# x42/meters.lv2

Measured on NVIDIA H100. Metric: audio-samples/sec/GPU (48 kHz stereo, 8192-ch batch) EBU R128 + true-peak, higher is better.
Workload: dtype f32

## Files before the change

### meters.lv2_b200/csrc/tpk.cu

```cuda
#include <math.h>
#include <stdlib.h>
#include <algorithm>
#include "common.cuh"
#include "tpk_internal.cuh"
#include "ebu_kw.cuh"

namespace b200m {

constexpr int TPK_THREADS = 128;

__constant__ float c_tp_tab[120];

struct TpkParams {
    float w1, w2, w3, g;
    float omega, fall; int hold;
    float kq[4], kc4;
};

struct TpkState {
    float *hist;
    float *tp_z1, *tp_z2, *tp_m, *tp_p; int *tp_res;
    float *km_z1, *km_z2, *km_rms, *km_peak, *km_fall; int *km_cnt, *km_fpp, *km_flag;
    unsigned* done_cnt;
    float* hist_alt;
// ... 1159 lines not shown
                    } else fir16<true> (w, xw, o, full0);
                }
                const int nv = min (4, len - 4 * q);
#pragma unroll
                for (int i = 0; i < 4; ++i)
                    if (i < nv) kpv.z = fmax3 (kpv.z, max3_abs (o[4 * i], o[4 * i + 1], o[4 * i + 2]), fabsf (o[4 * i + 3]));
            }
            if (c >= 2) bar_sync_2<BAR_EMPTY, TPK_THREADS> (b);
            if (act) {
                float4* d = reinterpret_cast<float4*> (&ob[b][r][0]);
#pragma unroll
                for (int i = 0; i < 4; ++i)
                    d[i * GPC + q] = make_float4 (fabsf (o[4 * i]), fabsf (o[4 * i + 1]), fabsf (o[4 * i + 2]), fabsf (o[4 * i + 3]));
                kp[b][r][q] = kpv;
            }
            bar_arrive_2<BAR_FULL, TPK_THREADS> (b);
        }
        {
            const int cl = nchunks - 1, base = (cl & (TPD_NSLOT - 1)) * TC + (nfram - cl * TC);
            for (int idx = ftid; idx < CH * 48; idx += TPD_FIR) {
                const int rr = idx / 48, j = idx - 48 * rr;
                if (c0 + rr < n_chan) st.hist[(size_t)(c0 + rr) * 48 + j] = xs[rr][base + j];
            }
        }
    } else {
        const int tch = lane & 15, filt = lane >> 4;
        const int chs = min (c0 + tch, n_chan - 1);
        const bool live = (c0 + tch) < n_chan;
        const int res = st.tp_res[chs];
        float m = res ? 0.0f : st.tp_m[chs];
        float p = res ? 0.0f : st.tp_p[chs];
        float z;
        { const float a = filt ? st.tp_z2[chs] : st.tp_z1[chs]; z = a > 20 ? 20 : (a < 0 ? 0 : a); }
        const float wf = filt ? prm.w2 : prm.w1;
        const float omw = __fsub_rn (1.0f, wf), wq = __fsub_rn (1.0f, omw), omw3 = __fmul_rn (omw, prm.w3);
        float kz1 = 0, kz2 = 0, kt = 0;
        if (KM) {
            const float a = st.km_z1[chs], b = st.km_z2[chs];
            kz1 = a > 50 ? 50 : (a < 0 ? 0 : a);
            kz2 = b > 50 ? 50 : (b < 0 ? 0 : b);
        }
        const float om4 = __fmul_rn (4.0f, prm.omega), nkc4 = -prm.kc4;
        auto step = [&] (const float4 v4) {
            if (FMA) {
                const float zd = __fmul_rn (z, prm.w3);
                z = fmaxf (zd, fmaf (omw3, z, __fmul_rn (wq, v4.x)));
                z = fmaxf (z, fmaf (omw, z, __fmul_rn (wq, v4.y)));
                z = fmaxf (z, fmaf (omw, z, __fmul_rn (wq, v4.z)));
                z = fmaxf (z, fmaf (omw, z, __fmul_rn (wq, v4.w)));
            } else {
                z = __fmul_rn (z, prm.w3);
                if (v4.x > z) z = __fadd_rn (z, __fmul_rn (wf, __fsub_rn (v4.x, z)));
                if (v4.y > z) z = __fadd_rn (z, __fmul_rn (wf, __fsub_rn (v4.y, z)));
                if (v4.z > z) z = __fadd_rn (z, __fmul_rn (wf, __fsub_rn (v4.z, z)));
                if (v4.w > z) z = __fadd_rn (z, __fmul_rn (wf, __fsub_rn (v4.w, z)));
            }
            m = fmaxf (m, __fadd_rn (z, __shfl_xor_sync (0xffffffffu, z, 16)));
        };
        for (int c = 0; c < nchunks; ++c) {
            const int b = c & 1, s0 = c * TC, len = min (TC, nfram - s0);
            bar_sync_2<BAR_FULL, TPK_THREADS> (b);
            const float4* b4 = reinterpret_cast<const float4*> (&ob[b][tch][0]);
            const float4* k4 = &kp[b][tch][0];
            const float4* x4 = reinterpret_cast<const float4*> (&xs[tch][48 + (c & (TPD_NSLOT - 1)) * TC]);
            const int ng = len >> 2;
#pragma unroll 2
            for (int g = 0; g < ng; ++g) {
                const float4 v0 = b4[g], v1 = b4[GPC + g], v2 = b4[2 * GPC + g], v3 = b4[3 * GPC + g];
                const float4 k = k4[g];
                step (v0); step (v1); step (v2); step (v3);
                p = fmaxf (p, k.z);
                if (KM && s0 + 4 * g + 4 <= km_n) {
                    if (FMA) {
                        kz1 = __fadd_rn (kz1, fmaf (nkc4, kz1, k.x));
                        kz2 = fmaf (om4, __fsub_rn (kz1, kz2), kz2);
                        kt = fmaxf (kt, k.y);
                    } else {
                        const float4 xv = x4[g];
                        const float vv[4] = {xv.x, xv.y, xv.z, xv.w};
#pragma unroll
                        for (int i = 0; i < 4; ++i) {
                            const float sq = __fmul_rn (vv[i], vv[i]);
                            if (kt < sq) kt = sq;
                            kz1 = __fadd_rn (kz1, __fmul_rn (prm.omega, __fsub_rn (sq, kz1)));
                        }
                        kz2 = __fadd_rn (kz2, __fmul_rn (om4, __fsub_rn (kz1, kz2)));
                    }
                }
            }
            if (4 * ng < len) {
                for (int j = 4 * ng; j < len; ++j) step (b4[(j & 3) * GPC + (j >> 2)]);
                p = fmaxf (p, k4[ng].z);
            }
            if (c + 2 < nchunks) bar_arrive_2<BAR_EMPTY, TPK_THREADS> (b);
        }
        if (live) {
            if (filt) st.tp_z2[chs] = __fadd_rn (z, 1e-20f);
            else {
                st.tp_z1[chs] = __fadd_rn (z, 1e-20f);
                m = __fmul_rn (m, prm.g);
                if (res) { st.tp_m[chs] = m; st.tp_p[chs] = p; st.tp_res[chs] = 0; }
                else {
                    if (m > st.tp_m[chs]) st.tp_m[chs] = m;
                    if (p > st.tp_p[chs]) st.tp_p[chs] = p;
                }
                if (KM) {
                    if (isnan (kz1)) kz1 = 0;
                    if (isnan (kz2)) kz2 = 0;
                    if (!finitef_ (kt)) kt = 0;
                    st.km_z1[chs] = __fadd_rn (kz1, 1e-20f);
                    st.km_z2[chs] = __fadd_rn (kz2, 1e-20f);
                    const float sr = __fsqrt_rn (__fmul_rn (2.0f, kz2));
                    const float tr = __fsqrt_rn (kt);
                    if (st.km_flag[chs]) { st.km_rms[chs] = sr; st.km_flag[chs] = 0; }
                    else if (sr > st.km_rms[chs]) st.km_rms[chs] = sr;
                    float pk = st.km_peak[chs]; int cnt = st.km_cnt[chs];
                    if (tr >= pk) { pk = tr; cnt = prm.hold; }
                    else if (cnt > 0) cnt -= nfram;
                    else { pk = __fmul_rn (pk, prm.fall); pk = __fadd_rn (pk, 1e-10f); }
                    st.km_peak[chs] = pk; st.km_cnt[chs] = cnt;
                    st.km_fall[chs] = prm.fall; st.km_fpp[chs] = nfram;
                }
            }
        }
    }
}

constexpr int TCF_XPITCH = 308;
constexpr int TCF_XSTAGES = 8;
constexpr int TCF_BLBO = 96 * 16;
constexpr int TCF_BBYTES = 16 * TCF_BLBO;
constexpr int TCF_SMEM = TCF_BBYTES + TCF_XSTAGES * 8 * TCF_XPITCH * 4 + 256;
constexpr int TCF_THREADS = 288;
constexpr int TCF_CONSUMERS = 256;

B200M_DEV uint32_t tcf_smem_u32 (const void* p) { return (uint32_t)__cvta_generic_to_shared (p); }
B200M_DEV uint64_t tcf_desc (uint32_t saddr, uint32_t lbo, uint32_t sbo)
{
    return (uint64_t)((saddr & 0x3FFFFu) >> 4) | ((uint64_t)(lbo >> 4) << 16) | ((uint64_t)(sbo >> 4) << 32);
}
B200M_DEV void tcf_wait (uint32_t bar, uint32_t parity)
{
    uint32_t ok = 0;
    while (!ok) asm volatile ("{ .reg .pred p; mbarrier.try_wait.parity.shared::cta.b64 p, [%1], %2; selp.u32 %0, 1, 0, p; }" : "=r"(ok) : "r"(bar), "r"(parity) : "memory");
}
B200M_DEV void tcf_arrive (uint32_t bar) { asm volatile ("mbarrier.arrive.shared::cta.b64 _, [%0];" :: "r"(bar) : "memory"); }
B200M_DEV void tcf_wgmma_n96 (float (&d)[48], const uint32_t (&a)[4], uint64_t db, uint32_t scale_d)
{
    asm volatile ("{\n\t.reg .pred p;\n\tsetp.ne.b32 p, %53, 0;\n\t"
                  "wgmma.mma_async.sync.aligned.m64n96k8.f32.tf32.tf32 {%0, %1, %2, %3, %4, %5, %6, %7, %8, %9, %10, %11, %12, %13, %14, %15, %16, %17, %18, %19, %20, %21, %22, %23, %24, %25, %26, %27, %28, %29, %30, %31, %32, %33, %34, %35, %36, %37, %38, %39, %40, %41, %42, %43, %44, %45, %46, %47}, {%48, %49, %50, %51}, %52, p, 1, 1;\n\t}\n"
                  : "+f"(d[0]), "+f"(d[1]), "+f"(d[2]), "+f"(d[3]), "+f"(d[4]), "+f"(d[5]), "+f"(d[6]), "+f"(d[7]), "+f"(d[8]), "+f"(d[9]), "+f"(d[10]), "+f"(d[11]), "+f"(d[12]), "+f"(d[13]), "+f"(d[14]), "+f"(d[15]), "+f"(d[16]), "+f"(d[17]), "+f"(d[18]), "+f"(d[19]), "+f"(d[20]), "+f"(d[21]), "+f"(d[22]), "+f"(d[23]), "+f"(d[24]), "+f"(d[25]), "+f"(d[26]), "+f"(d[27]), "+f"(d[28]), "+f"(d[29]), "+f"(d[30]), "+f"(d[31]), "+f"(d[32]), "+f"(d[33]), "+f"(d[34]), "+f"(d[35]), "+f"(d[36]), "+f"(d[37]), "+f"(d[38]), "+f"(d[39]), "+f"(d[40]), "+f"(d[41]), "+f"(d[42]), "+f"(d[43]), "+f"(d[44]), "+f"(d[45]), "+f"(d[46]), "+f"(d[47])
                  : "r"(a[0]), "r"(a[1]), "r"(a[2]), "r"(a[3]), "l"(db), "r"(scale_d) : "memory");
}
B200M_DEV void tcf_wgmma_n48 (float (&d)[48], const uint32_t (&a)[4], uint64_t db, uint32_t scale_d)
{
    asm volatile ("{\n\t.reg .pred p;\n\tsetp.ne.b32 p, %29, 0;\n\t"
                  "wgmma.mma_async.sync.aligned.m64n48k8.f32.tf32.tf32 {%0, %1, %2, %3, %4, %5, %6, %7, %8, %9, %10, %11, %12, %13, %14, %15, %16, %17, %18, %19, %20, %21, %22, %23}, {%24, %25, %26, %27}, %28, p, 1, 1;\n\t}\n"
                  : "+f"(d[0]), "+f"(d[1]), "+f"(d[2]), "+f"(d[3]), "+f"(d[4]), "+f"(d[5]), "+f"(d[6]), "+f"(d[7]), "+f"(d[8]), "+f"(d[9]), "+f"(d[10]), "+f"(d[11]), "+f"(d[12]), "+f"(d[13]), "+f"(d[14]), "+f"(d[15]), "+f"(d[16]), "+f"(d[17]), "+f"(d[18]), "+f"(d[19]), "+f"(d[20]), "+f"(d[21]), "+f"(d[22]), "+f"(d[23])
                  : "r"(a[0]), "r"(a[1]), "r"(a[2]), "r"(a[3]), "l"(db), "r"(scale_d) : "memory");
}

B200M_DEV void tcf_load (const float* xw, float (&v)[8][4])
{
#pragma unroll
    for (int s = 0; s < 8; ++s) { v[s][0] = xw[8 * s]; v[s][1] = xw[16 + 8 * s]; v[s][2] = xw[8 * s + 4]; v[s][3] = xw[16 + 8 * s + 4]; }
}
B200M_DEV float tcf_mask_p0 (float (&v)[8][4], int t, const int (&vj)[2], const int (&nin)[2])
{
    if (nin[1] < 64) {
#pragma unroll
        for (int s = 0; s < 8; ++s)
#pragma unroll
            for (int e = 0; e < 4; ++e)
                if (8 * s + t + 4 * (e >> 1) >= nin[e & 1]) v[s][e] = 0.0f;
    }
    float p0 = 0.0f;
#pragma unroll
    for (int s = 3; s < 5; ++s)
#pragma unroll
        for (int e = 0; e < 4; ++e)
            if (8 * (s - 3) + t + 4 * (e >> 1) < vj[e & 1]) p0 = fmaxf (p0, fabsf (v[s][e]));
    return p0;
}
B200M_DEV void tcf_split (const float (&v)[8][4], uint32_t (&ahi)[8][4], uint32_t (&alo)[8][4])
{
#pragma unroll
    for (int s = 0; s < 8; ++s)
#pragma unroll
        for (int e = 0; e < 4; ++e) {
            const uint32_t hbits = __float_as_uint (v[s][e]) & 0xffffe000u;
            ahi[s][e] = hbits; alo[s][e] = __float_as_uint (__fsub_rn (v[s][e], __uint_as_float (hbits)));
        }
}
B200M_DEV void tcf_mma (float (&d)[48], const uint32_t (&ahi)[8][4], const uint32_t (&alo)[8][4], uint32_t bb)
{
    asm volatile ("wgmma.fence.sync.aligned;" ::: "memory");
#pragma unroll
    for (int s = 0; s < 8; ++s) {
        const uint64_t db = tcf_desc (bb + 2 * s * TCF_BLBO, TCF_BLBO, 128);
        tcf_wgmma_n96 (d, ahi[s], db, s == 0 ? 0u : 1u);
        tcf_wgmma_n48 (d, alo[s], db, 1u);
    }
    asm volatile ("wgmma.commit_group.sync.aligned;" ::: "memory");
}
B200M_DEV void tcf_mma_wait () { asm volatile ("wgmma.wait_group.sync.aligned 0;" ::: "memory"); }
B200M_DEV float tcf_tile_max (const float (&d)[48], int t, const int (&vj)[2], float mx)
{
#pragma unroll
    for (int i = 0; i < 6; ++i)
#pragma unroll
        for (int e = 0; e < 2; ++e) {
            const int j = 8 * (i & 1) + 2 * t + e;
            if (j < vj[0]) mx = fmaxf (mx, fabsf (__fadd_rn (d[4 * i + e], d[4 * (i + 6) + e])));
            if (j < vj[1]) mx = fmaxf (mx, fabsf (__fadd_rn (d[4 * i + 2 + e], d[4 * (i + 6) + 2 + e])));
        }
    return mx;
}

template <int HOLD>
__global__ void __launch_bounds__ (TCF_THREADS, 1)
tpmax_tc_kernel (const float* __restrict__ in, size_t stride, int c_first, int n_chan, int nfram, int nchunks, const float* __restrict__ bcanon,
                 TpkState st, R128Hold r128)
{
    extern __shared__ __align__ (128) uint8_t tcf_smem[];
    uint8_t* sB = tcf_smem;
    float* xbuf = reinterpret_cast<float*> (tcf_smem + TCF_BBYTES);
    uint64_t* bars = reinterpret_cast<uint64_t*> (tcf_smem + TCF_BBYTES + TCF_XSTAGES * 8 * TCF_XPITCH * 4);
    uint64_t* xfull = bars; uint64_t* xempty = bars + TCF_XSTAGES;
    const int tid = threadIdx.x, warp = tid >> 5, lane = tid & 31;
    const int ngroups = (n_chan - c_first + 7) / 8;
    const int n_it = (int)blockIdx.x < ngroups ? ((ngroups - (int)blockIdx.x + (int)gridDim.x - 1) / (int)gridDim.x) * nchunks : 0;
    __shared__ unsigned s_gmax[8];
    if (tid < 8) s_gmax[tid] = 0u;

    for (int i = tid; i < TCF_BBYTES / 16; i += TCF_THREADS) reinterpret_cast<float4*> (sB)[i] = reinterpret_cast<const float4*> (bcanon)[i];
    if (tid == 0) {
        for (int i = 0; i < TCF_XSTAGES; ++i) {
            asm volatile ("mbarrier.init.shared::cta.b64 [%0], 1;" :: "r"(tcf_smem_u32 (&xfull[i])));
            asm volatile ("mbarrier.init.shared::cta.b64 [%0], %1;" :: "r"(tcf_smem_u32 (&xempty[i])), "n"(TCF_CONSUMERS));
        }
        asm volatile ("fence.mbarrier_init.release.cluster;" ::: "memory");
    }
    asm volatile ("fence.proxy.async.shared::cta;" ::: "memory");
    __syncthreads ();

    if (warp == 8) {
        if (lane == 0)
            for (int it = 0; it < n_it; ++it) {
                const int sg = it % TCF_XSTAGES;
                if (it >= TCF_XSTAGES) tcf_wait (tcf_smem_u32 (&xempty[sg]), (uint32_t)((it / TCF_XSTAGES - 1) & 1));
                const int gk = it / nchunks, chunk = it - gk * nchunks;
                const int c0 = c_first + ((int)blockIdx.x + gk * (int)gridDim.x) * 8, s0 = chunk * 256;
                const uint32_t xb = tcf_smem_u32 (xbuf + (size_t)sg * 8 * TCF_XPITCH), bar = tcf_smem_u32 (&xfull[sg]);
                const uint32_t nfl = (uint32_t)min (304, nfram - (s0 - 48));
                asm volatile ("mbarrier.arrive.expect_tx.shared::cta.b64 _, [%0], %1;" :: "r"(bar), "r"(8u * nfl * 4u) : "memory");
                for (int cc = 0; cc < 8; ++cc) {
                    const size_t ch = (size_t)min (c0 + cc, n_chan - 1);
                    const uint32_t dst = xb + (uint32_t)(cc * TCF_XPITCH * 4);
                    if (chunk == 0) {
                        asm volatile ("cp.async.bulk.shared::cluster.global.mbarrier::complete_tx::bytes [%0], [%1], %2, [%3];"
                                      :: "r"(dst), "l"(st.hist + ch * 48), "r"(192u), "r"(bar) : "memory");
                        asm volatile ("cp.async.bulk.shared::cluster.global.mbarrier::complete_tx::bytes [%0], [%1], %2, [%3];"
                                      :: "r"(dst + 192u), "l"(in + ch * stride), "r"((nfl - 48u) * 4u), "r"(bar) : "memory");
                    } else
                        asm volatile ("cp.async.bulk.shared::cluster.global.mbarrier::complete_tx::bytes [%0], [%1], %2, [%3];"
                                      :: "r"(dst), "l"(in + ch * stride + (s0 - 48)), "r"(nfl * 4u), "r"(bar) : "memory");
                }
            }
    } else {
        const int wg = warp >> 2, g = lane >> 2, t = lane & 3;
        const int tb0 = 8 * wg + 2 * (warp & 3);
        const uint32_t bb = tcf_smem_u32 (sB);
        for (int it = 0; it < n_it; ++it) {
            const int gk = it / nchunks, chunk = it - gk * nchunks;
            const int c0 = c_first + ((int)blockIdx.x + gk * (int)gridDim.x) * 8, s0 = chunk * 256;
            const int sg = it % TCF_XSTAGES;
            tcf_wait (tcf_smem_u32 (&xfull[sg]), (uint32_t)((it / TCF_XSTAGES) & 1));
            const float* xt = xbuf + (size_t)sg * 8 * TCF_XPITCH;
            const float* xw = xt + g * TCF_XPITCH + 16 * tb0 + t;
            float v[8][4];
            tcf_load (xw, v);
            if (chunk == nchunks - 1 && tid < 96) {
                const int rr = tid / 12, k4 = (tid - 12 * rr) * 4;
                if (c0 + rr < n_chan)
                    *reinterpret_cast<float4*> (st.hist_alt + (size_t)(c0 + rr) * 48 + k4) = *reinterpret_cast<const float4*> (xt + rr * TCF_XPITCH + (nfram - s0) + k4);
            }
            tcf_arrive (tcf_smem_u32 (&xempty[sg]));
            int vj[2], nin[2];
#pragma unroll
            for (int h = 0; h < 2; ++h) {
                vj[h] = min (16, max (0, nfram - (s0 + 16 * (tb0 + h))));
                nin[h] = nfram - (s0 - 48) - 16 * (tb0 + h);
            }
            const float p0 = tcf_mask_p0 (v, t, vj, nin);
            uint32_t ahi[8][4], alo[8][4];
            tcf_split (v, ahi, alo);
            float d[48];
            tcf_mma (d, ahi, alo, bb);
            tcf_mma_wait ();
            float mx = tcf_tile_max (d, t, vj, p0);
            mx = fmaxf (mx, __shfl_xor_sync (0xffffffffu, mx, 1));
            mx = fmaxf (mx, __shfl_xor_sync (0xffffffffu, mx, 2));
            if (t == 0 && mx > 0.0f) atomicMax (&s_gmax[g], __float_as_uint (mx));
            if (chunk == nchunks - 1) {
                asm volatile ("bar.sync 1, %0;" :: "n"(TCF_CONSUMERS) : "memory");
                if (warp == 0) {
                    const int cc = c0 + lane;
                    const bool own = lane < 8 && cc < n_chan;
                    float mm = 0.0f;
                    if (lane < 8) { const float bm = __uint_as_float (s_gmax[lane]); s_gmax[lane] = 0u; mm = bm; }
                    if (own) {
                        const float m0 = st.tp_res[cc] ? 0.0f : st.tp_m[cc];
                        if (!(mm > m0)) mm = m0;
                        st.tp_m[cc] = mm;
                    }
                    if (r128.tpmax) r128_group_hold<HOLD> (r128, st, mm, cc, own);
                }
                asm volatile ("bar.sync 1, %0;" :: "n"(TCF_CONSUMERS) : "memory");
            }
        }
    }
    __syncthreads ();
    if (r128.tpmax && tid == 0) {
        const unsigned dn = atomicAdd (st.done_cnt, 1u);
        if (dn == gridDim.x - 1) { *st.done_cnt = 0u; asm volatile ("griddepcontrol.wait;" ::: "memory"); }
    }
}

constexpr int R128F_CH = 128, R128F_PITCH = 116, R128F_SLOTS = 3, R128F_WARPS = 12;
constexpr int R128F_STAGE_BYTES = R128F_CH * R128F_PITCH * 4;
constexpr int R128F_SMEM = 128 + TCF_BBYTES + R128F_SLOTS * R128F_STAGE_BYTES + 64 + R128F_CH * 4;
static_assert (EBU_TILE == 64, "a stage is one K1 tile");

struct R128fRing {
    uint8_t* stage; uint32_t full, cnt;
    const CUtensorMap* tmap; const float* in; size_t stride; const float* hist; int nch, nfram, ntiles, nslabs, slab;

    B200M_DEV uint8_t* slot (int j) const { return stage + (j % R128F_SLOTS) * R128F_STAGE_BYTES; }
    B200M_DEV void wait (int j) const { tcf_wait (full + 8 * (j % R128F_SLOTS), (uint32_t)(j / R128F_SLOTS) & 1u); }
    B200M_DEV void produce (int j, int lane) const
    {
        const int i = j / ntiles, t = j - i * ntiles;
        if (i >= nslabs) return;
        const int c0 = ((int)blockIdx.x + i * (int)gridDim.x) * slab;
        const uint32_t dst = smem_u32 (slot (j)), bar = full + 8 * (j % R128F_SLOTS);
        if (t == 0) {
            const uint32_t nb = (uint32_t)min (68, nfram) * 4u;
            if (lane == 0) asm volatile ("mbarrier.arrive.expect_tx.shared::cta.b64 _, [%0], %1;" :: "r"(bar), "r"((uint32_t)R128F_CH * (192u + nb)) : "memory");
            __syncwarp ();
            asm volatile ("fence.proxy.async.shared::cta;" ::: "memory");
            for (int r = lane; r < R128F_CH; r += 32) {
                const size_t ch = (size_t)min (c0 + r, nch - 1);
                const uint32_t d = dst + (uint32_t)(r * R128F_PITCH * 4);
                asm volatile ("cp.async.bulk.shared::cluster.global.mbarrier::complete_tx::bytes [%0], [%1], %2, [%3];"
                              :: "r"(d), "l"(hist + ch * 48), "r"(192u), "r"(bar) : "memory");
                asm volatile ("cp.async.bulk.shared::cluster.global.mbarrier::complete_tx::bytes [%0], [%1], %2, [%3];"
                              :: "r"(d + 192u), "l"(in + ch * stride), "r"(nb), "r"(bar) : "memory");
            }
        } else if (lane == 0) {
            asm volatile ("fence.proxy.async.shared::cta;" ::: "memory");
            asm volatile ("mbarrier.arrive.expect_tx.shared::cta.b64 _, [%0], %1;" :: "r"(bar), "r"((uint32_t)R128F_STAGE_BYTES) : "memory");
            asm volatile ("cp.async.bulk.tensor.2d.shared::cluster.global.tile.mbarrier::complete_tx::bytes [%0], [%1, {%2, %3}], [%4];"
                          :: "r"(dst), "l"(tmap), "r"(64 * t - 48), "r"(c0), "r"(bar) : "memory");
        }
    }
    B200M_DEV void release (int j, int lane) const
    {
// ... 288 lines not shown
            const auto k = h->imm && h->fma ? tpmax_kernel_for<true, true> (hold) : h->imm ? tpmax_kernel_for<true, false> (hold) : tpmax_kernel_for<false, false> (hold);
            B200M_CUDA (cudaLaunchKernelEx (&cfg, k, d_in, stride, cf, ce, (int)nfram, nchunks, aligned, h->elide0, h->st, h->d_dbg, r128));
            swap_hist = true;
        }
        else if (tp && tp_mode == B200M_TP_MODE_MAX) { if (km) TPK_GO (8, 256, true, true, true, false); else TPK_GO (8, 256, true, true, false, false); }
        else if (tp && h->split && h->d_scr) {
            const int nslab = ((int)nfram + (int)h->slab - 1) / (int)h->slab;
            const int ngrp = (ce - cf + TPF_CH - 1) / TPF_CH, nb16 = (ce - cf + 15) / 16;
            for (int sidx = 0; sidx < nslab; ++sidx) {
                const int sb0 = sidx * (int)h->slab, sl_len = std::min ((int)h->slab, (int)nfram - sb0), b = sidx & 1;
                float4* scr = h->d_scr + (size_t)b * h->n_chan * h->slab + (size_t)cf * h->slab;
                if (sidx >= 2) B200M_CUDA (cudaStreamWaitEvent (st, h->ev_bal[b], 0));
                const int nch = (sl_len + TPF_TC - 1) / TPF_TC;
                if (h->imm && h->fma) tpfir_kernel<true, true><<<ngrp * nch, blk, 0, st>>> (d_in, stride, cf, ce, (int)nfram, sb0, sl_len, aligned, h->elide0, h->st, scr, (int)h->slab, h->d_dbg, h->d_tl, h->tl_next);
                else if (h->imm) tpfir_kernel<true, false><<<ngrp * nch, blk, 0, st>>> (d_in, stride, cf, ce, (int)nfram, sb0, sl_len, aligned, h->elide0, h->st, scr, (int)h->slab, h->d_dbg, h->d_tl, h->tl_next);
                else tpfir_kernel<false, false><<<ngrp * nch, blk, 0, st>>> (d_in, stride, cf, ce, (int)nfram, sb0, sl_len, aligned, h->elide0, h->st, scr, (int)h->slab, h->d_dbg, h->d_tl, h->tl_next);
                B200M_CUDA (cudaEventRecord (h->ev_fir[b], st));
                B200M_CUDA (cudaStreamWaitEvent (h->sb, h->ev_fir[b], 0));
                const int first = sidx == 0, last = sidx == nslab - 1;
                if (km && drp.rms_sum) tpbal_kernel<true, true><<<nb16, 64, 0, h->sb>>> (scr, (int)h->slab, d_in, stride, cf, ce, (int)h->n_chan, (int)nfram, sb0, sl_len, first, last, aligned, 1, prm, h->st, drp, h->d_tl, h->tl_next + 1);
                else if (km) tpbal_kernel<true, false><<<nb16, 64, 0, h->sb>>> (scr, (int)h->slab, d_in, stride, cf, ce, (int)h->n_chan, (int)nfram, sb0, sl_len, first, last, aligned, 1, prm, h->st, drp, h->d_tl, h->tl_next + 1);
                else tpbal_kernel<false, false><<<nb16, 64, 0, h->sb>>> (scr, (int)h->slab, d_in, stride, cf, ce, (int)h->n_chan, (int)nfram, sb0, sl_len, first, last, aligned, 1, prm, h->st, drp, h->d_tl, h->tl_next + 1);
                B200M_CUDA (cudaEventRecord (h->ev_bal[b], h->sb));
                B200M_LAUNCHED (2);
                if (h->d_tl) h->tl_next = (h->tl_next + 2) % 4096;
            }
            B200M_CUDA (cudaStreamWaitEvent (st, h->ev_bal[(nslab - 1) & 1], 0));
            if (nslab >= 2) B200M_CUDA (cudaStreamWaitEvent (st, h->ev_bal[(nslab - 2) & 1], 0));
            swap_hist = true;
            continue;
        }
        else if (tp && h->dec && h->imm && !h->d_dbg && !drp.rms_sum) {
            const unsigned grid = (unsigned)((ce - cf + TPD_CH - 1) / TPD_CH);
            if (h->fma) {
                if (km) tpdec_kernel<true, true><<<grid, blk, 0, st>>> (d_in, stride, cf, ce, (int)nfram, aligned, h->elide0, prm, h->st);
                else tpdec_kernel<false, true><<<grid, blk, 0, st>>> (d_in, stride, cf, ce, (int)nfram, aligned, h->elide0, prm, h->st);
            } else {
                if (km) tpdec_kernel<true, false><<<grid, blk, 0, st>>> (d_in, stride, cf, ce, (int)nfram, aligned, h->elide0, prm, h->st);
                else tpdec_kernel<false, false><<<grid, blk, 0, st>>> (d_in, stride, cf, ce, (int)nfram, aligned, h->elide0, prm, h->st);
            }
        }
        else if (tp && h->wide && (ce - cf) >= h->wide_min) {
            if (km) { if (drp.rms_sum) TPK_GO (64, 32, true, false, true, true); else TPK_GO (64, 32, true, false, true, false); } else TPK_GO (64, 32, true, false, false, false);
        }
        else if (tp) { if (km) { if (drp.rms_sum) TPK_GO (16, 64, true, false, true, true); else TPK_GO (16, 64, true, false, true, false); } else TPK_GO (16, 64, true, false, false, false); }
        else tpk_kernel<16, 64, false, false, true, false, false><<<(ce - cf + 15) / 16, blk, TpkGeom<16, 64, false>::BYTES, st>>> (d_in, stride, cf, ce, (int)nfram, aligned, h->elide0, prm, h->st, h->d_dbg, r128, drp);
#undef TPK_GO
        B200M_LAUNCHED (1);
    }
    if (swap_hist) { float* t = h->st.hist; h->st.hist = h->st.hist_alt; h->st.hist_alt = t; }
    B200M_CUDA (cudaGetLastError ());
    return 0;
}

static int tpk_process (b200m_tpk* h, const float* d_in, size_t stride, uint32_t nfram, uint32_t tp_mode, cudaStream_t st)
{
    const uint32_t bounds[2] = {0, h->n_chan};
    return tpk_process_sliced (h, d_in, stride, nfram, tp_mode, st, 1, bounds, nullptr, R128Hold {}, false, h->dr_on ? &h->dr : nullptr);
}

constexpr uint32_t R128F_MIN_CH = 10240;

float* tpk_hist (b200m_tpk* h) { return h->st.hist; }

bool tpk_r128_fused_ok (const b200m_tpk* h, const float* d_in, size_t stride, uint32_t nfram)
{
    return (h->flags & B200M_TPK_TRUEPEAK) && !(h->flags & B200M_TPK_KMETER) && h->chunked && h->tc && h->fma && h->imm && h->d_btc && !h->d_dbg
        && (uintptr_t)d_in % 16 == 0 && stride % 4 == 0 && nfram % 4 == 0 && h->n_chan >= R128F_MIN_CH;
}

#define R128F_K(N) {r128_fused_kernel<N, false>, r128_fused_kernel<N, true>}
static const decltype (&r128_fused_kernel<2, false>) r128f_kernels[5][2] = {R128F_K (1), R128F_K (2), R128F_K (3), R128F_K (4), R128F_K (5)};
#undef R128F_K

int tpk_r128_fused (b200m_tpk* h, const EbuK1Args& a, float* r128_tpmax, cudaStream_t st)
{
    if (a.nchans != (int)h->n_chan) return set_err (B200M_E_INVAL, "r128: EBU and true-peak banks disagree on the channel count");
    const int nchan = a.nchans / a.n_inst;
    if (nchan < 1 || nchan > 5 || nchan * a.n_inst != a.nchans) return set_err (B200M_E_INVAL, "r128: %d channels per instance", nchan);
    CUtensorMap tm;
    if (!ebu_tma_map (&tm, a.in, a.stride, h->n_chan, (uint32_t)a.nfram, R128F_PITCH, R128F_CH, false))
        return set_err (B200M_E_CUDA, "r128: the driver rejected the input block's tensor map");
    const int slab = 4 * (32 / nchan) * nchan, nslabs = ((int)h->n_chan + slab - 1) / slab;
    r128f_kernels[nchan - 1][a.ck.fph ? 1 : 0]<<<std::min (nslabs, h->n_sm), R128F_WARPS * 32, R128F_SMEM, st>>> (
        tm, a.in, a.stride, (int)h->n_chan, a.nfram, h->d_btc, h->st, r128_tpmax, a.cf, a.ck, a.fragm_f, a.zst, a.frpwr, a.fragpw, a.n_inst);
    B200M_LAUNCHED (1);
    B200M_CUDA (cudaGetLastError ());
    float* t = h->st.hist; h->st.hist = h->st.hist_alt; h->st.hist_alt = t;
    return 0;
}

extern "C" {

int b200m_design_tpk (float fsamp, float w[4], float ctab[120], float km[2])
{
    if (!(fsamp >= 1000.0f)) return set_err (B200M_E_INVAL, "bad argument");
    TpkParams p; float t[120]; tpk_design (fsamp, p, t);
    if (w) { w[0] = p.w1; w[1] = p.w2; w[2] = p.w3; w[3] = p.g; }
    if (ctab) memcpy (ctab, t, sizeof (t));
    if (km) { km[0] = p.omega; km[1] = (float)p.hold; }
    return 0;
}

int b200m_tpk_create (b200m_tpk** out, int device, uint32_t n_chan, float fsamp, uint32_t flags)
{
    if (!out) return set_err (B200M_E_INVAL, "NULL out pointer");
    *out = nullptr;
    if (n_chan == 0 || !(fsamp >= 1000.0f) || !(flags & 3u) || (flags & ~3u)) return set_err (B200M_E_INVAL, "bad n_chan/fsamp/flags");
    if (b200m_device_count () <= 0) return set_err (B200M_E_NODEVICE, "no CUDA device: b200meters has no CPU path");
    DeviceGuard g (device);
    if (!g.ok) return set_err (B200M_E_NODEVICE, "cannot select CUDA device %d", device);
    b200m_tpk* h = new (std::nothrow) b200m_tpk;
    if (!h) return set_err (B200M_E_NOMEM, "host allocation failed");
    h->device = device; h->n_chan = n_chan; h->flags = flags; h->fsamp = fsamp;
    tpk_design (fsamp, h->prm, h->ctab);
    h->imm = memcmp (h->ctab, h_zita_lit, sizeof (h->ctab)) == 0;
    if (const char* v = getenv ("B200M_TPK_IMM")) h->imm = h->imm && atoi (v);
    {
        double S = 0.0;
        for (int i = 0; i < 24; ++i) S += (i == 23 ? 0.0 : fabs ((double)h->ctab[i])) + fabs ((double)h->ctab[96 + i]);
        h->elide0 = h->ctab[23] == 1.0f && S <= 7.71e-16;
    }
    if (const char* v = getenv ("B200M_TPK_ELIDE0")) h->elide0 = h->elide0 && atoi (v);
    if (const char* v = getenv ("B200M_TPK_PRECISION")) h->fma = (strcmp (v, "fma") == 0) && h->imm && h->ctab[23] == 1.0f;
    cudaError_t e = cudaMemcpyToSymbol (c_tp_tab, h->ctab, sizeof (h->ctab));
    if (e == cudaSuccess) e = cudaFuncSetAttribute (tpk_kernel<8, 256, true, true, false, true, false, true>, cudaFuncAttributePreferredSharedMemoryCarveout, cudaSharedmemCarveoutMaxShared);
    if (e == cudaSuccess) e = cudaFuncSetAttribute (tpk_kernel<8, 256, true, true, false, true, false, false>, cudaFuncAttributePreferredSharedMemoryCarveout, cudaSharedmemCarveoutMaxShared);
    if (e == cudaSuccess) e = cudaFuncSetAttribute (tpk_kernel<8, 256, true, true, false, false, false, false>, cudaFuncAttributePreferredSharedMemoryCarveout, cudaSharedmemCarveoutMaxShared);
    if (e == cudaSuccess) e = cudaFuncSetAttribute (tpdec_kernel<true, true>, cudaFuncAttributePreferredSharedMemoryCarveout, cudaSharedmemCarveoutMaxShared);
    if (e == cudaSuccess) e = cudaFuncSetAttribute (tpdec_kernel<false, true>, cudaFuncAttributePreferredSharedMemoryCarveout, cudaSharedmemCarveoutMaxShared);
    if (e == cudaSuccess) e = cudaFuncSetAttribute (tpdec_kernel<true, false>, cudaFuncAttributePreferredSharedMemoryCarveout, cudaSharedmemCarveoutMaxShared);
    if (e == cudaSuccess) e = cudaFuncSetAttribute (tpdec_kernel<false, false>, cudaFuncAttributePreferredSharedMemoryCarveout, cudaSharedmemCarveoutMaxShared);
    for (const int hold : R128_HOLDS)
        for (const auto k : {tpmax_kernel_for<true, true> (hold), tpmax_kernel_for<true, false> (hold), tpmax_kernel_for<false, false> (hold)})
            if (e == cudaSuccess) e = cudaFuncSetAttribute (k, cudaFuncAttributePreferredSharedMemoryCarveout, cudaSharedmemCarveoutMaxShared);
    auto A = [&] (void** p, size_t bytes) { if (e == cudaSuccess) { e = cudaMalloc (p, bytes); if (e == cudaSuccess) e = cudaMemset (*p, 0, bytes); } };
    const size_t n = n_chan;
    A ((void**)&h->st.hist, n * 48 * sizeof (float));
    A ((void**)&h->st.tp_z1, n * 4); A ((void**)&h->st.tp_z2, n * 4); A ((void**)&h->st.tp_m, n * 4); A ((void**)&h->st.tp_p, n * 4);
    A ((void**)&h->st.tp_res, n * 4);
    A ((void**)&h->st.km_z1, n * 4); A ((void**)&h->st.km_z2, n * 4); A ((void**)&h->st.km_rms, n * 4); A ((void**)&h->st.km_peak, n * 4);
    A ((void**)&h->st.km_fall, n * 4); A ((void**)&h->st.km_cnt, n * 4); A ((void**)&h->st.km_fpp, n * 4); A ((void**)&h->st.km_flag, n * 4);
    A ((void**)&h->d_res, n * sizeof (b200m_tpk_result));
    A ((void**)&h->st.done_cnt, 16);
    A ((void**)&h->st.hist_alt, n * 48 * sizeof (float));
    A ((void**)&h->st.blk_max, n * 4); A ((void**)&h->st.grp_cnt, n * 4);
    if (const char* v = getenv ("B200M_TPK_CHUNKED")) h->chunked = atoi (v) != 0;
    if (const char* v = getenv ("B200M_TPK_TC")) h->tc = atoi (v) != 0;
    if ((flags & B200M_TPK_TRUEPEAK) && h->imm && e == cudaSuccess) {
        float* hb = new (std::nothrow) float[TCF_BBYTES / 4];
        if (hb) {
            memset (hb, 0, TCF_BBYTES);
            for (int n = 0; n < 48; ++n) for (int k = 0; k < 64; ++k) {
                const int ph = n / 16 + 1, j = n % 16, d = j + 48 - k;
                const float c = (d >= 0 && d <= 47) ? (d >= 24 ? h->ctab[24 * ph + 47 - d] : h->ctab[24 * (4 - ph) + d]) : 0.0f;
                uint32_t u; memcpy (&u, &c, 4); u &= 0xffffe000u; float hi; memcpy (&hi, &u, 4);
                const size_t off = ((size_t)(k / 4) * TCF_BLBO + (size_t)n * 16 + (size_t)(k % 4) * 4) / 4;
                hb[off] = hi; hb[off + 48 * 4] = c - hi;
            }
            e = cudaMalloc ((void**)&h->d_btc, TCF_BBYTES);
            if (e == cudaSuccess) e = cudaMemcpy (h->d_btc, hb, TCF_BBYTES, cudaMemcpyHostToDevice);
            delete[] hb;
        }
        for (const int hold : R128_HOLDS) {
            if (e == cudaSuccess) e = cudaFuncSetAttribute (tpmax_tc_kernel_for (hold), cudaFuncAttributeMaxDynamicSharedMemorySize, TCF_SMEM);
            if (e == cudaSuccess) e = cudaFuncSetAttribute (tpmax_tc_kernel_for (hold), cudaFuncAttributePreferredSharedMemoryCarveout, cudaSharedmemCarveoutMaxShared);
        }
        for (const auto& kp : r128f_kernels)
            for (const auto k : kp) if (e == cudaSuccess) e = cudaFuncSetAttribute (k, cudaFuncAttributeMaxDynamicSharedMemorySize, R128F_SMEM);
        if (e == cudaSuccess) e = cudaDeviceGetAttribute (&h->n_sm, cudaDevAttrMultiProcessorCount, device);
    }
    if (const char* v = getenv ("B200M_TPK_DEC")) h->dec = atoi (v) != 0;
    h->split = 0;
    if (const char* v = getenv ("B200M_TPK_SPLIT")) { const int q = atoi (v); h->split = q >= 2 ? 1 : (q == 1 ? n_chan >= 512 : 0); }
    A ((void**)&h->st.tmp, 7 * n * sizeof (float));
    { const char* v = getenv ("B200M_TPK_STAGGER"); if (v && atoi (v) != 0) A ((void**)&h->st.sm_arr, 256 * sizeof (unsigned)); }
    if ((flags & B200M_TPK_TRUEPEAK) && h->split) {
        uint32_t slab = 64;
        while (slab < B200M_MAX_BLOCK && (size_t)2 * n * (2 * slab) * 16 <= ((size_t)64 << 20)) slab *= 2;
        if (const char* v = getenv ("B200M_TPK_SLAB")) { const int q = atoi (v); if (q >= 64 && q <= (int)B200M_MAX_BLOCK && q % 64 == 0) slab = (uint32_t)q; }
        h->slab = slab;
        if (const char* v = getenv ("B200M_TPK_TIMELINE")) if (atoi (v) && e == cudaSuccess) {
            e = cudaMallocManaged ((void**)&h->d_tl, 4096 * 2 * sizeof (unsigned long long));
            if (e == cudaSuccess) for (int i = 0; i < 4096; ++i) { h->d_tl[2 * i] = ~0ull; h->d_tl[2 * i + 1] = 0ull; }
        }
        A ((void**)&h->d_scr, (size_t)2 * n * slab * sizeof (float4));
        int prio_lo = 0, prio_hi = 0;
        if (e == cudaSuccess) e = cudaDeviceGetStreamPriorityRange (&prio_lo, &prio_hi);
        if (e == cudaSuccess) e = cudaStreamCreateWithPriority (&h->sb, cudaStreamNonBlocking, prio_hi);
        for (int i = 0; i < 2; ++i) {
            if (e == cudaSuccess) e = cudaEventCreateWithFlags (&h->ev_fir[i], cudaEventDisableTiming);
            if (e == cudaSuccess) e = cudaEventCreateWithFlags (&h->ev_bal[i], cudaEventDisableTiming);
        }
    }
    if (const char* v = getenv ("B200M_TPK_WIDE")) {
        const int w = atoi (v); h->wide = w != 0;
        if (w > 1) h->wide_min = w;
        else if (e == cudaSuccess) { int nsm = 0; e = cudaDeviceGetAttribute (&nsm, cudaDevAttrMultiProcessorCount, device); h->wide_min = 64 * nsm; }
    }
#define TPK_WATTR(KMF, DRF, FMAF) if (e == cudaSuccess) e = cudaFuncSetAttribute (tpk_kernel<64, 32, true, false, KMF, true, DRF, FMAF>, cudaFuncAttributeMaxDynamicSharedMemorySize, (int)TpkGeom<64, 32, true>::BYTES)
    TPK_WATTR (true, true, true); TPK_WATTR (true, true, false); TPK_WATTR (true, false, true); TPK_WATTR (true, false, false); TPK_WATTR (false, false, true); TPK_WATTR (false, false, false);
#undef TPK_WATTR
    if (e == cudaSuccess) e = cudaFuncSetAttribute (tpk_kernel<64, 32, true, false, true, false, true, false>, cudaFuncAttributeMaxDynamicSharedMemorySize, (int)TpkGeom<64, 32, true>::BYTES);
    if (e == cudaSuccess) e = cudaFuncSetAttribute (tpk_kernel<64, 32, true, false, true, false, false, false>, cudaFuncAttributeMaxDynamicSharedMemorySize, (int)TpkGeom<64, 32, true>::BYTES);
    if (e == cudaSuccess) e = cudaFuncSetAttribute (tpk_kernel<64, 32, true, false, false, false, false, false>, cudaFuncAttributeMaxDynamicSharedMemorySize, (int)TpkGeom<64, 32, true>::BYTES);
    if (e == cudaSuccess) e = cudaStreamCreateWithFlags (&h->own, cudaStreamNonBlocking);
    if (e == cudaSuccess) {
        tpk_reset_kernel<<<(n_chan + 127) / 128, 128>>> ((int)n_chan, -1, B200M_TPK_TRUEPEAK, h->st, nullptr, 0, 1);
        B200M_LAUNCHED (1);
        e = cudaDeviceSynchronize ();
    }
    if (e != cudaSuccess) { int rc = cuda_fail (e, "tpk_create", __FILE__, __LINE__); b200m_tpk_destroy (h); return rc; }
    *out = h;
    return 0;
}

int b200m_tpk_destroy (b200m_tpk* h)
{
    if (!h) return 0;
    DeviceGuard g (h->device);
    cudaDeviceSynchronize ();
    void* ps[] = {h->st.hist, h->st.tp_z1, h->st.tp_z2, h->st.tp_m, h->st.tp_p, h->st.tp_res, h->st.km_z1, h->st.km_z2, h->st.km_rms,
                  h->st.km_peak, h->st.km_fall, h->st.km_cnt, h->st.km_fpp, h->st.km_flag, h->d_res, h->d_dbg, h->st.done_cnt, h->st.hist_alt, h->st.blk_max, h->st.grp_cnt, h->st.tmp, h->d_scr, h->st.sm_arr, h->d_tl, h->d_btc};
    for (void* p : ps) cudaFree (p);
    if (h->sb) cudaStreamDestroy (h->sb);
    for (int i = 0; i < 2; ++i) { if (h->ev_fir[i]) cudaEventDestroy (h->ev_fir[i]); if (h->ev_bal[i]) cudaEventDestroy (h->ev_bal[i]); }
    h->stage.release ();
    if (h->own) cudaStreamDestroy (h->own);
    delete h;
    return 0;
}

int b200m_tpk_process_device (b200m_tpk* h, const float* d_in, size_t stride, uint32_t nfram, uint32_t tp_mode, void* stream)
{
    if (int rc = check_block_args (h, d_in, stride, nfram)) return rc;
    if (tp_mode > 1) return set_err (B200M_E_INVAL, "bad tp_mode %u", tp_mode);
    DeviceGuard g (h->device);
    h->last_host = false;
    return tpk_process (h, d_in, stride, nfram, tp_mode, (cudaStream_t)stream);
}

int b200m_tpk_process_host (b200m_tpk* h, const float* in, size_t stride, uint32_t nfram, uint32_t tp_mode)
{
    if (int rc = check_block_args (h, in, stride, nfram)) return rc;
    if (tp_mode > 1) return set_err (B200M_E_INVAL, "bad tp_mode %u", tp_mode);
    DeviceGuard g (h->device);
    B200M_ENTER_HOST_PATH (h);
    if (h->stage.ensure (h->n_chan, nfram)) return set_err (B200M_E_NOMEM, "staging buffer allocation failed");
    B200M_CUDA (cudaMemcpy2DAsync (h->stage.d, h->stage.cap * sizeof (float), in, stride * sizeof (float),
                                   (size_t)nfram * sizeof (float), h->n_chan, cudaMemcpyHostToDevice, h->own));
    h->last_host = true;
    return tpk_process (h, h->stage.d, h->stage.cap, nfram, tp_mode, h->own);
}

int b200m_tpk_set_precision (b200m_tpk* h, int mode)
{
    if (!h || (mode != B200M_PREC_EXACT && mode != B200M_PREC_FMA)) return set_err (B200M_E_INVAL, "bad argument");
    if (mode == B200M_PREC_FMA && !(h->imm && h->ctab[23] == 1.0f)) return set_err (B200M_E_UNSUPPORTED, "tolerance mode needs the literal zita table");
    h->fma = mode == B200M_PREC_FMA;
    return 0;
}
int b200m_tpk_precision (const b200m_tpk* h) { return h ? (h->fma ? B200M_PREC_FMA : B200M_PREC_EXACT) : B200M_E_INVAL; }

int b200m_tpk_read_device (b200m_tpk* h, void* stream)
{
    if (!h) return set_err (B200M_E_INVAL, "NULL handle");
    DeviceGuard g (h->device);
    tpk_read_kernel<<<(h->n_chan + 255) / 256, 256, 0, tpk_stream (h, stream)>>> ((int)h->n_chan, h->flags, h->st, h->d_res);
    B200M_LAUNCHED (1);
    B200M_CUDA (cudaGetLastError ());
    return 0;
}

int b200m_tpk_results (b200m_tpk* h, b200m_tpk_result* out, void* stream)
{
    if (!h || !out) return set_err (B200M_E_INVAL, "NULL argument");
    DeviceGuard g (h->device);
    cudaStream_t st = tpk_stream (h, stream);
    B200M_CUDA (cudaMemcpyAsync (out, h->d_res, h->n_chan * sizeof (b200m_tpk_result), cudaMemcpyDeviceToHost, st));
    B200M_CUDA (cudaStreamSynchronize (st));
    return 0;
}

int b200m_tpk_reset (b200m_tpk* h, int32_t chan, void* stream)
{
    if (!h || chan >= (int32_t)h->n_chan) return set_err (B200M_E_INVAL, "bad argument");
    DeviceGuard g (h->device);
    tpk_reset_kernel<<<(h->n_chan + 127) / 128, 128, 0, tpk_stream (h, stream)>>> ((int)h->n_chan, chan, h->flags, h->st, nullptr, 0, 1);
    B200M_LAUNCHED (1);
    B200M_CUDA (cudaGetLastError ());
    return 0;
}

int b200m_tpk_clear (b200m_tpk* h, int32_t chan, void* stream)
{
    if (!h || chan >= (int32_t)h->n_chan) return set_err (B200M_E_INVAL, "bad argument");
    DeviceGuard g (h->device);
    tpk_reset_kernel<<<(h->n_chan + 127) / 128, 128, 0, tpk_stream (h, stream)>>> ((int)h->n_chan, chan, h->flags | 4u, h->st, nullptr, 0, 1);
    B200M_LAUNCHED (1);
    B200M_CUDA (cudaGetLastError ());
    return 0;
}

int b200m_tpk_reset_kmeter (b200m_tpk* h, void* stream)
{
    if (!h) return set_err (B200M_E_INVAL, "NULL handle");
    DeviceGuard g (h->device);
    tpk_reset_kernel<<<(h->n_chan + 127) / 128, 128, 0, tpk_stream (h, stream)>>> ((int)h->n_chan, -1, h->flags & B200M_TPK_KMETER, h->st, nullptr, 0, 1);
    B200M_LAUNCHED (1);
    B200M_CUDA (cudaGetLastError ());
    return 0;
// ... 123 lines not shown
```

Baseline: 187.4 billion.

## Skip zero coefficient blocks in true-peak wgmma by banding first and last k-steps

Reorders the packed FIR coefficient matrix columns so that in the first and last k-slices, where the polyphase band is partly zero, smaller wgmma shapes (n48/n24) cover only the nonzero columns. The accumulator register mapping and the tile max reduction are remapped to match. This cuts tensor-core work in the edge k-steps of the split hi/lo TF32 product. The price is a more intricate descriptor and column layout, which raises the risk of indexing errors.

```diff
diff --git a/meters.lv2_b200/csrc/tpk.cu b/meters.lv2_b200/csrc/tpk.cu
--- a/meters.lv2_b200/csrc/tpk.cu
+++ b/meters.lv2_b200/csrc/tpk.cu
@@ -1335,11 +1335,22 @@
                   : "+f"(d[0]), "+f"(d[1]), "+f"(d[2]), "+f"(d[3]), "+f"(d[4]), "+f"(d[5]), "+f"(d[6]), "+f"(d[7]), "+f"(d[8]), "+f"(d[9]), "+f"(d[10]), "+f"(d[11]), "+f"(d[12]), "+f"(d[13]), "+f"(d[14]), "+f"(d[15]), "+f"(d[16]), "+f"(d[17]), "+f"(d[18]), "+f"(d[19]), "+f"(d[20]), "+f"(d[21]), "+f"(d[22]), "+f"(d[23]), "+f"(d[24]), "+f"(d[25]), "+f"(d[26]), "+f"(d[27]), "+f"(d[28]), "+f"(d[29]), "+f"(d[30]), "+f"(d[31]), "+f"(d[32]), "+f"(d[33]), "+f"(d[34]), "+f"(d[35]), "+f"(d[36]), "+f"(d[37]), "+f"(d[38]), "+f"(d[39]), "+f"(d[40]), "+f"(d[41]), "+f"(d[42]), "+f"(d[43]), "+f"(d[44]), "+f"(d[45]), "+f"(d[46]), "+f"(d[47])
                   : "r"(a[0]), "r"(a[1]), "r"(a[2]), "r"(a[3]), "l"(db), "r"(scale_d) : "memory");
 }
+template <int O>
 B200M_DEV void tcf_wgmma_n48 (float (&d)[48], const uint32_t (&a)[4], uint64_t db, uint32_t scale_d)
 {
+    float* h = d + O;
     asm volatile ("{\n\t.reg .pred p;\n\tsetp.ne.b32 p, %29, 0;\n\t"
                   "wgmma.mma_async.sync.aligned.m64n48k8.f32.tf32.tf32 {%0, %1, %2, %3, %4, %5, %6, %7, %8, %9, %10, %11, %12, %13, %14, %15, %16, %17, %18, %19, %20, %21, %22, %23}, {%24, %25, %26, %27}, %28, p, 1, 1;\n\t}\n"
-                  : "+f"(d[0]), "+f"(d[1]), "+f"(d[2]), "+f"(d[3]), "+f"(d[4]), "+f"(d[5]), "+f"(d[6]), "+f"(d[7]), "+f"(d[8]), "+f"(d[9]), "+f"(d[10]), "+f"(d[11]), "+f"(d[12]), "+f"(d[13]), "+f"(d[14]), "+f"(d[15]), "+f"(d[16]), "+f"(d[17]), "+f"(d[18]), "+f"(d[19]), "+f"(d[20]), "+f"(d[21]), "+f"(d[22]), "+f"(d[23])
+                  : "+f"(h[0]), "+f"(h[1]), "+f"(h[2]), "+f"(h[3]), "+f"(h[4]), "+f"(h[5]), "+f"(h[6]), "+f"(h[7]), "+f"(h[8]), "+f"(h[9]), "+f"(h[10]), "+f"(h[11]), "+f"(h[12]), "+f"(h[13]), "+f"(h[14]), "+f"(h[15]), "+f"(h[16]), "+f"(h[17]), "+f"(h[18]), "+f"(h[19]), "+f"(h[20]), "+f"(h[21]), "+f"(h[22]), "+f"(h[23])
+                  : "r"(a[0]), "r"(a[1]), "r"(a[2]), "r"(a[3]), "l"(db), "r"(scale_d) : "memory");
+}
+template <int O>
+B200M_DEV void tcf_wgmma_n24 (float (&d)[48], const uint32_t (&a)[4], uint64_t db, uint32_t scale_d)
+{
+    float* h = d + O;
+    asm volatile ("{\n\t.reg .pred p;\n\tsetp.ne.b32 p, %17, 0;\n\t"
+                  "wgmma.mma_async.sync.aligned.m64n24k8.f32.tf32.tf32 {%0, %1, %2, %3, %4, %5, %6, %7, %8, %9, %10, %11}, {%12, %13, %14, %15}, %16, p, 1, 1;\n\t}\n"
+                  : "+f"(h[0]), "+f"(h[1]), "+f"(h[2]), "+f"(h[3]), "+f"(h[4]), "+f"(h[5]), "+f"(h[6]), "+f"(h[7]), "+f"(h[8]), "+f"(h[9]), "+f"(h[10]), "+f"(h[11])
                   : "r"(a[0]), "r"(a[1]), "r"(a[2]), "r"(a[3]), "l"(db), "r"(scale_d) : "memory");
 }
 
@@ -1378,11 +1389,17 @@
 B200M_DEV void tcf_mma (float (&d)[48], const uint32_t (&ahi)[8][4], const uint32_t (&alo)[8][4], uint32_t bb)
 {
     asm volatile ("wgmma.fence.sync.aligned;" ::: "memory");
-#pragma unroll
-    for (int s = 0; s < 8; ++s) {
+    const uint32_t b0 = bb, b7 = bb + 14 * TCF_BLBO;
+    tcf_wgmma_n48<12> (d, ahi[0], tcf_desc (b0 + 24 * 16, TCF_BLBO, 128), 0u);
+    tcf_wgmma_n24<12> (d, alo[0], tcf_desc (b0 + 24 * 16, TCF_BLBO, 128), 1u);
+    tcf_wgmma_n24<0> (d, ahi[7], tcf_desc (b7, TCF_BLBO, 128), 0u);
+    tcf_wgmma_n24<36> (d, ahi[7], tcf_desc (b7 + 72 * 16, TCF_BLBO, 128), 0u);
+    tcf_wgmma_n24<0> (d, alo[7], tcf_desc (b7, TCF_BLBO, 128), 1u);
+#pragma unroll
+    for (int s = 1; s < 7; ++s) {
         const uint64_t db = tcf_desc (bb + 2 * s * TCF_BLBO, TCF_BLBO, 128);
-        tcf_wgmma_n96 (d, ahi[s], db, s == 0 ? 0u : 1u);
-        tcf_wgmma_n48 (d, alo[s], db, 1u);
+        tcf_wgmma_n96 (d, ahi[s], db, 1u);
+        tcf_wgmma_n48<0> (d, alo[s], db, 1u);
     }
     asm volatile ("wgmma.commit_group.sync.aligned;" ::: "memory");
 }
@@ -1393,9 +1410,10 @@
     for (int i = 0; i < 6; ++i)
 #pragma unroll
         for (int e = 0; e < 2; ++e) {
-            const int j = 8 * (i & 1) + 2 * t + e;
-            if (j < vj[0]) mx = fmaxf (mx, fabsf (__fadd_rn (d[4 * i + e], d[4 * (i + 6) + e])));
-            if (j < vj[1]) mx = fmaxf (mx, fabsf (__fadd_rn (d[4 * i + 2 + e], d[4 * (i + 6) + 2 + e])));
+            const int j = 8 * (i / 3) + 2 * t + e;
+            const int ih = i < 3 ? i + 3 : i - 3, il = i + 6;
+            if (j < vj[0]) mx = fmaxf (mx, fabsf (__fadd_rn (d[4 * ih + e], d[4 * il + e])));
+            if (j < vj[1]) mx = fmaxf (mx, fabsf (__fadd_rn (d[4 * ih + 2 + e], d[4 * il + 2 + e])));
         }
     return mx;
 }
@@ -1990,11 +2008,12 @@
         if (hb) {
             memset (hb, 0, TCF_BBYTES);
             for (int n = 0; n < 48; ++n) for (int k = 0; k < 64; ++k) {
-                const int ph = n / 16 + 1, j = n % 16, d = j + 48 - k;
+                const int ph = n / 16 + 1, j = n % 16, d = j + 48 - k, q = 8 * (ph - 1) + j % 8;
+                const int chi = j < 8 ? 24 + q : q, clo = j < 8 ? 48 + q : 72 + q;
                 const float c = (d >= 0 && d <= 47) ? (d >= 24 ? h->ctab[24 * ph + 47 - d] : h->ctab[24 * (4 - ph) + d]) : 0.0f;
                 uint32_t u; memcpy (&u, &c, 4); u &= 0xffffe000u; float hi; memcpy (&hi, &u, 4);
-                const size_t off = ((size_t)(k / 4) * TCF_BLBO + (size_t)n * 16 + (size_t)(k % 4) * 4) / 4;
-                hb[off] = hi; hb[off + 48 * 4] = c - hi;
+                const size_t off = ((size_t)(k / 4) * TCF_BLBO + (size_t)(k % 4) * 4) / 4;
+                hb[off + chi * 4] = hi; hb[off + clo * 4] = c - hi;
             }
             e = cudaMalloc ((void**)&h->d_btc, TCF_BBYTES);
             if (e == cudaSuccess) e = cudaMemcpy (h->d_btc, hb, TCF_BBYTES, cudaMemcpyHostToDevice);
```

Result: no change. 191.3 billion, median of 6 (+2.1%).
